# precice/dealii-adapter

Hardware: AMD Instinct MI355X
Metric: DoF-updates/sec per Newmark step (assembly+CG), 3D Q2 ~5M DoFs (higher is better)
Workload: dtype f64

## Files before the change

dealii-adapter_amd/csrc/mi_ctx.cpp:

```cpp
#include <hip/hip_runtime.h>
#include <rccl/rccl.h>

#include <algorithm>
#include <chrono>
#include <cmath>
#include <cstdarg>
#include <cstdio>
#include <cstdlib>
#include <cstring>
#include <functional>
#include <string>
#include <vector>

#include "mi_internal.h"

namespace mi_detail
{
  std::string g_create_error;

  enum
  {
    SC_RZ0 = 0,
    SC_RZ1 = 1,
    SC_TOL = 2,
// ... 120 lines not shown
      L.begin[c] = int32_t(m.ncells);
    L.ncol = m.ncolours;
    const int npc = m.npc, np1 = m.np1;
    for (int64_t pos = 0; pos < m.ncells; ++pos)
      {
        int col = 0;
        for (int c = 1; c < 8; ++c)
          col += pos >= L.begin[c] ? 1 : 0;
        const mi::CellLatticeRow &R = rows[size_t(col)];
        const uint32_t r   = uint32_t(pos - L.begin[col]);
        const uint32_t rz  = uint32_t((uint64_t(r) * R.magic_mxy) >> 42);
        const uint32_t rem = r - rz * uint32_t(R.mxy);
        const uint32_t ry  = uint32_t((uint64_t(rem) * R.magic_mx) >> 42);
        const uint32_t rx  = rem - ry * uint32_t(R.mx);
        const int32_t  n0  = R.base + int32_t(rx) * L.sx + int32_t(ry) * L.sy + int32_t(rz) * L.sz;
        for (int a = 0; a < npc; ++a)
          {
            const int i = a % np1, j = (a / np1) % np1, k = a / (np1 * np1);
            if (m.conn[size_t(pos) * npc + a] != n0 + i + j * L.nn0 + k * L.nn01)
              return mi::CellLattice{};
          }
      }
    return L;
  }

  mi::AsmParams asm_params(mi_ctx *c)
  {
    mi::AsmParams p{};
    static const bool asm_lat = mi::exp_env("MI_ASM_CELL_LATTICE") && atoi(mi::exp_env("MI_ASM_CELL_LATTICE")) != 0;
    if (asm_lat)
      p.lat = c->lat;
    p.conn   = c->d_conn;
    p.cverts = c->d_cverts;
    p.off    = c->d_off;
    p.rowinfo = reinterpret_cast<const int2 *>(c->d_rowinfo);
    p.cmask  = c->d_cmask;
    p.tab1d  = c->d_tab;
    p.u      = c->vec(MI_V_TOTAL_DISPLACEMENT);
    p.du     = c->vec(MI_V_SOLUTION_DELTA);
    p.acc    = c->vec(MI_V_ACCELERATION);
    p.stress = c->vec(MI_V_EXTERNAL_STRESS);
    p.rhs    = c->vec(MI_V_SYSTEM_RHS);
    p.vals   = c->d_vals;
    p.zero_blk  = uint32_t(c->mesh.nvalblocks() + 1);
    p.trash_blk = uint32_t(c->mesh.nvalblocks() + 2);
    p.mu     = c->mat.mu;
// ... 143 lines not shown

  int element_form(const mi_ctx *c)
  {
    if (!c->ke_valid)
      return 0;
    if (c->d_qrec_q3)
      return 2;
    if (c->d_qrec && (c->ebe == 2 || !c->d_ke))
      return 2;
    return c->d_ke ? 1 : 0;
  }

  bool smoother_runs_q27(const mi_ctx *c)
  {
    return c->smoother_points == 3 && c->qrec27_valid && element_form(c) == 2 && c->mf_slots && c->d_mf_yc &&
           !c->active_sell_vals && (c->mf_fine || (c->ebe != 0 && c->precond_storage == 64)) &&
           !(c->smoother_precision == 32 && c->qrec32_valid);
  }

  bool mf_gather_fusable(const mi_ctx *c)
  {
    return element_form(c) == 2 && c->ebe == 2 && c->mf_slots && c->d_mf_yc && c->precond_storage == 64 &&
           !c->active_sell_vals && c->d_dinv_blk;
  }

  mi::MfParams mf_params(const mi_ctx *c)
  {
    mi::MfParams f{};
    f.conn = c->d_conn, f.first = c->d_node_first, f.cmask = c->d_cmask, f.cverts = c->d_cverts, f.cellbox = c->d_cellbox;
    f.tab1d = c->d_tab, f.tab27 = c->d_tab27, f.lat = c->lat, f.qrec27 = c->d_qrec27;
    f.mu = c->mat.mu, f.kappa = c->kappa, f.mass = c->alpha[1] * c->mat.rho;
    return f;
  }

  void enqueue_spmv(mi_ctx *c, const double *x, double *y, const double *dotv, double *partials, const int32_t *done,
                    int part, bool smoother, const ChebFusion *cheb)
  {
    const int  kind       = element_form(c);
    const bool mf_all     = c->mf_fine && !c->active_sell_vals;
    const bool ebe_for_cg = dotv && (c->cg_operator == 1 || mf_all) && kind && !c->active_sell_vals && !cheb;
    const bool cheb_ok    = !cheb || (cheb->inplace && smoother && mf_gather_fusable(c));
    if (ebe_for_cg || (kind && cheb_ok && !dotv && !c->active_sell_vals &&
                       (mf_all || (smoother ? (c->ebe != 0 && c->precond_storage == 64) : (c->spmv_variant == 4 || c->unassembled_now)))))
      {
        const bool q3  = c->d_qrec_q3 != nullptr;
        const bool q27 = smoother && !ebe_for_cg && smoother_runs_q27(c);
// ... 61 lines not shown
                    return;
                  }
                layers(0, zlo, false);
                layers(zhi, nzl, false);
              }
            else if (q3)
              {
                const int t = sample ? tic(c0, MI_T_EBE_LAUNCH, true) : -1;
                mi::launch_mf_spmv_q3(f, int32_t(c->mesh.ncells), c->stream, t >= 0 ? c0->stamps[size_t(t)].a : nullptr,
                                      t >= 0 ? c0->stamps[size_t(t)].b : nullptr);
              }
            else if (q27)
              {
                const int t = sample ? tic(c0, MI_T_EBE_LAUNCH, true) : -1;
                mi::launch_mf_spmv27(f, int32_t(c->mesh.ncells), c->stream, t >= 0 ? c0->stamps[size_t(t)].a : nullptr,
                                     t >= 0 ? c0->stamps[size_t(t)].b : nullptr);
              }
            else
              {
                const int t = sample ? tic(c0, MI_T_EBE_LAUNCH, true) : -1;
                mi::launch_mf_spmv(f, 0, int32_t(c->mesh.ncells), c->stream, t >= 0 ? c0->stamps[size_t(t)].a : nullptr,
                                   t >= 0 ? c0->stamps[size_t(t)].b : nullptr);
              }
            if (cheb && cheb->xnext)
              mi::launch_mf_gather_cheb3(f, cheb->b, cheb->dinv6, cheb->xprev, x, cheb->xnext, cheb->c1, cheb->c2, c->own0 / 3,
                                         c->own_n / 3, c->stream);
            else if (cheb)
              mi::launch_mf_gather_cheb(f, cheb->b, cheb->dinv, cheb->d, const_cast<double *>(x), y, cheb->c1, cheb->c2,
                                        c->own0 / 3, c->own_n / 3, c->stream);
            else if (ebe_for_cg)
              mi::launch_mf_gather_dot(f, int64_t(c->mesh.nnodes) * 3, dotv, partials, c->grid_gdot, c->own0, c->own_n, c->stream);
            else
              mi::launch_mf_gather(f, int64_t(c->mesh.nnodes) * 3, c->stream);
          }
        else
        for (int col = 0; col < c->mesh.ncolours; ++col)
          {
            const int32_t cnt = int32_t(c->mesh.colour_begin[col + 1] - c->mesh.colour_begin[col]);
            const int     t   = (sample && cnt > 0) ? tic(c0, MI_T_EBE_LAUNCH, true) : -1;
            if (kind == 2)
              mi::launch_mf_spmv(f, c->mesh.colour_begin[col], cnt, c->stream, t >= 0 ? c0->stamps[size_t(t)].a : nullptr,
                                 t >= 0 ? c0->stamps[size_t(t)].b : nullptr);
            else
              mi::launch_ebe_spmv(e, c->mesh.colour_begin[col], cnt, c->stream, t >= 0 ? c0->stamps[size_t(t)].a : nullptr,
                                  t >= 0 ? c0->stamps[size_t(t)].b : nullptr);
          }
        if (ebe_for_cg && !one_launch)
          mi::launch_dot_partials(dotv + c->own0, y + c->own0, c->own_n, partials, c->grid_vec, c->stream);
        return;
      }
    if (c->spmv_variant == 3 || c->spmv_variant == 4 || c->active_sell_vals)
      {
        refresh_vals32(c);
        mi::SellParams p   = sell_params(c, x, y, dotv, partials, done);
        if (smoother && c->precond_storage == 32 && c->d_sell_vals32 && !c->active_sell_vals)
          p.vals32 = c->d_sell_vals32;
// ... 367 lines not shown
      layout = 1;
    c->slots_layout = layout;
    if (layout)
      {
        src.resize(dst.size());
        std::vector<int32_t> place(dst.size());
        for (size_t k = 0; k < dst.size(); ++k)
          place[k] = int32_t(k);
        if (layout == 2)
          for (int col = 0; col < c->lat.ncol; ++col)
            {
              const mi::CellLatticeRow &R  = c->lat_rows_host[size_t(col)];
              const int64_t             b0 = c->lat.begin[col], b1 = c->lat.begin[col + 1];
              for (int64_t e = b0; e < b1; ++e)
                {
                  const int64_t r = e - b0, row = r / R.mx, rx = r - row * R.mx;
                  for (int a = 0; a < 27; ++a)
                    place[size_t(e) * 27 + a] = int32_t((b0 + row * R.mx) * 27 + int64_t(a / 3) * 3 * R.mx + rx * 3 + a % 3);
                }
            }
        for (size_t k = 0; k < dst.size(); ++k)
          src[size_t(dst[k])] = place[k];
        dst = place;
      }
    const bool cell_major = layout != 0;
    int rc = upload(c, &c->d_mf_dst, dst);
    if (rc == MI_OK)
      rc = upload(c, &c->d_mf_slot_base, base);
    if (rc == MI_OK && cell_major)
      rc = upload(c, &c->d_mf_src, src);
    if (rc)
      return rc;
    if (!c->d_mf_yc)
      HIPCHK(c, hipMalloc((void **)&c->d_mf_yc, size_t(nc) * npc * 3 * sizeof(double)));
    
    return MI_OK;
  }

  int alloc_records27(mi_ctx *c)
  {
    if (c->d_qrec27 || c->smoother_points != 3)
      return MI_OK;
    mi::Tables1D t3;
    t3.build(2, 3);
    const int rc = upload(c, &c->d_tab27, t3.packed());
    if (rc)
// ... 1877 lines not shown
            {
              const int rq = alloc_point_records(m);
              if (rq)
                return rq;
            }
          if (!m->d_node_first)
            {
              const int rc = upload(m, &m->d_node_first, m->mesh.node_first);
              if (rc)
                return rc;
            }
          m->ebe      = value;
          m->ke_valid = false;
        }
      else if (k == "mg_scale_lmax_percent" && value >= 10 && value <= 400)
        {
          if (m == c->team->members[0])
            mg_scale_estimates(*c->team, 0.01 * value);
        }
      else if (k == "mf_single_launch" && (value == 0 || value == 1))
        m->mf_slots = value;
      else if (k == "xcd_remap" && (value == 0 || value == 1))
        m->xcd_remap = value;
      else if (k == "cell_lattice" && (value == 0 || value == 1))
        m->lat = value ? m->lat_built : mi::CellLattice{};
      else if (k == "sell_unroll" && value >= -2 && value <= 8 && value != 0)
        m->sell_unroll = value;
      else if (k == "spmv_grid" && value >= 1 && value + m->grid_spmv_bnd <= MAX_PART)
        {
          m->split_int = m->split_bnd = false;
          if (m->mesh.sell_nslices_interior > 0)
            m->grid_spmv_int = value;
          else
            m->grid_spmv_bnd = value;
          m->grid_spmv = m->grid_spmv_int + m->grid_spmv_bnd;
        }
      else if (k == "sell_icol" && (value == 0 || value == 1))
        m->sell_icol = value;
      else if (k == "small_cg" && (value == 0 || value == 1))
        m->small_cg = value;
      else if (k == "halo_overlap" && (value == 0 || value == 1))
        c->team->overlap = value;
      else if (k == "asm_variant" && ((value >= 0 && value <= 2) || value == 9))
        m->asm_variant = value;
      else if (k == "mg_refresh_every" && value >= 1 && value <= 1000)
        m->mg_refresh_every = value;
// ... 89 lines not shown
               0;
  else if (k == "mf_single_launch")
    *value = (m->mf_slots && m->d_mf_yc) ? 1 : 0;
  else if (k == "fine_level")
    *value = m->mf_fine;
  else if (k == "mf_diag_lag")
    *value = m->mf_diag_lag;
  else if (k == "smoother_quadrature")
    *value = m->smoother_points;
  else if (k == "smoother_quadrature_active")
    *value = smoother_runs_q27(m) ? 3 : 4;
  else if (k == "experiments")
#ifdef MI_EXPERIMENTS
    *value = 1;
#else
    *value = 0;
#endif
  else if (k == "sell_icol")
    *value = m->sell_icol;
  else if (k == "asm_variant")
    *value = m->asm_variant;
  else if (k == "cell_lattice")
    *value = m->lat.ncol > 0 ? 1 : 0;
  else if (k == "cut_axis")
    *value = c->team->size > 1 ? c->team->amap.ext_axis[c->team->dim - 1] + 1 : 0;
  else if (k == "cg_speculate")
    *value = m->cg_speculate;
  else if (k == "smoother_precision")
    *value = m->smoother_precision;
  else if (k == "cg_single_reduction")
    *value = m->cg_single_reduction;
  else if (k == "mg_distributed_levels")
    *value = mg_distributed_levels(m);
  else if (k == "cg_single_reduction_active")
    *value = (m->cg_single_reduction == 1 || (m->cg_single_reduction < 0 && c->team->size > 1)) ? 1 : 0;
  else if (k == "cg_speculate_margin")
    *value = m->cg_speculate_margin;
  else if (k == "halo_skip")
    *value = c->team->halo_skip;
  else if (k == "precond")
    *value = m->precond;
  else if (k == "spmv_variant")
    *value = m->spmv_variant;
  else if (k == "count_scalar_allreduce")
    *value = int(c->team->n_scalar_allreduce);
  else if (k == "count_scalar_allreduce_cg")
// ... 174 lines not shown
```

dealii-adapter_amd/csrc/mi_internal.h:

```cpp
#pragma once
#include <hip/hip_runtime.h>

#include <cstdint>
#include <functional>
#include <memory>
#include <string>
#include <vector>

#include "../../include/mi_elasticity.h"
#include "mi_kernels.h"
#include "mi_mesh.hpp"

namespace mi_detail
{
  constexpr int MAX_PART = 16384;
  constexpr int CG_BATCH = 16;

  enum
  {
    W_R = 0,
    W_P,
    W_Q,
    W_DINV,
    W_Z,
// ... 88 lines not shown
  bool      want_dinv_blk = false;
  double   *d_ke = nullptr;
  uint32_t *d_node_first = nullptr;
  float    *d_qrec32 = nullptr;
  int       smoother_precision = 64;
  int       smoother_points = 3;
  double   *d_qrec27 = nullptr;
  double   *d_tab27  = nullptr;
  bool      qrec27_valid = false;
  int       spmv_as_smoother = 0;
  bool      qrec32_valid = false;
  double   *d_qrec = nullptr;
  double   *d_mf_yc = nullptr;
  int32_t  *d_mf_dst = nullptr;
  int32_t  *d_mf_slot_base = nullptr;
  int32_t  *d_mf_src = nullptr;
  int       slots_layout = 0;
  int       slots_cell_major = -1;
  int       mf_slots = 1;
  mi::CellLattice lat;
  mi::CellLattice lat_built;
  mi::CellLatticeRow *d_lat_rows = nullptr;
  std::vector<mi::CellLatticeRow> lat_rows_host;
  double   *d_cellbox = nullptr;
  bool      ke_valid = false;
  int64_t   ebe_products = 0;
  static constexpr int NPRED = 4;
  double   *d_pred[NPRED][2] = {}, *d_pred_saved[NPRED][2] = {};
  int       pred_count[NPRED] = {}, pred_count_saved[NPRED] = {}, solves_this_step = 0;
  int       cg_operator = 0;
  int       cg_warm_start = 0;
  int       cg_fused_dot = 1;
  int       correct_face_F = 0;
  int       cg_r0_unassembled = 1;
  bool      unassembled_now = false;
  int64_t   mg_dist_nodes = -1;
  int64_t   mg_coarsest = -1, mg_dense = -1;
  int       cg_single_reduction = -1;
  int       cg_speculate_margin = 0;
  int       cg_speculate = 1;
  int       pred_its[NPRED] = {};
  int       mf_fine = 0;
  double   *d_qrec_q3 = nullptr;
  int       mf_point_slots = 1;
  int       mf_diag_lag = 0;
  bool      mf_diag_fresh = false;
// ... 50 lines not shown
  bool                  mg_stale = true;
  bool                  mg_force = true;
  int                   asm_variant = 0;
  int                   asm_box_geometry = 1;
  int                   mg_lag   = 1;
  int                   mg_refresh_every = 8, mg_steps_since_refresh = 0, mg_its_ref = 0;
  int64_t               n_mg_refresh = 0;

  double *vec(int which) { return d_vecs + size_t(which) * size_t(n); }
  double *work(int which) { return d_work + size_t(which) * size_t(n); }
  double *part(int which) { return d_part + size_t(which) * mi_detail::MAX_PART; }
};

namespace mi_detail
{
  int  fail(mi_ctx *c, int code, const char *fmt, ...);
  int  tic(mi_ctx *c, int cls, bool ext = false);
  void toc(mi_ctx *c, int id);
  int  sync(mi_ctx *c);
  int            direct_prepare(mi_ctx *c);
  int            direct_factor_solve(mi_ctx *c, const double *vals, const double *b, double *x, bool factor, bool solve);
  void           refresh_vals32(mi_ctx *c);
  int            element_form(const mi_ctx *c);
  bool           mf_gather_fusable(const mi_ctx *c);
  mi::SellParams sell_params(mi_ctx *c, const double *x, double *y, const double *dotv, double *partials,
                             const int32_t *done);
  void enqueue_spmv(mi_ctx *c, const double *x, double *y, const double *dotv, double *partials, const int32_t *done,
                    int part = 0, bool smoother = false, const ChebFusion *cheb = nullptr);
  int  set_precond_storage(mi_ctx *c, int bits);
  int  cg_run(mi_ctx *c, int x_id, int b_id, double tol, int64_t max_it, int *its, double *res, bool x_is_zero = false,
              bool scale_start = false,
              int expected_its = 0);
  int  team_size(const mi_ctx *c);
  void linear_destroy(mi_ctx *c);
  int  create_member(Team &T, const mi_mesh_desc *md, const mi_material_desc *mat, const mi_newmark_desc *nm, int rank,
                     mi_ctx **out);
  void destroy_team(Team *T);
  int  enqueue_assembly(mi_ctx *c, bool residual_only = false);
  int  ensure_element_tangents(mi_ctx *c);
  int  mg_setup(mi_ctx *c);
  void mg_reset_estimates(Team &T);
  void mg_scale_estimates(Team &T, double f);
  void mg_destroy(mi_ctx *c);
  int  mg_update(Team &T);
  int  mg_distributed_levels(const mi_ctx *c);
  int  mg_apply(Team &T);
// ... 39 lines not shown
```

dealii-adapter_amd/csrc/mi_kernels.h:

```cpp
#pragma once
#include <hip/hip_runtime.h>
#include <stdint.h>

#include <stdlib.h>

namespace mi
{
#ifdef MI_EXPERIMENTS
  inline const char *exp_env(const char *name) { return getenv(name); }
#else
  inline const char *exp_env(const char *) { return nullptr; }
#endif

  struct CellLatticeRow
  {
    int32_t  mx, mxy, base, pz;
    uint64_t magic_mx, magic_mxy;
  };
  struct CellLattice
  {
    int32_t               ncol = 0;
    int32_t               begin[9] = {};
    int32_t               sx = 0, sy = 0, sz = 0, nn0 = 0, nn01 = 0;
    const CellLatticeRow *rows = nullptr;
  };

  struct AsmParams
  {
    const int32_t  *conn;
    const double   *cverts;
    const uint16_t *off;
    const int2     *rowinfo;
    const uint8_t  *cmask;
    const double   *tab1d;
    const double   *u, *du, *acc, *stress;
    double         *rhs;
    double         *vals;
    uint32_t        zero_blk, trash_blk;
    double          mu, kappa, rho, alpha1;
    double          body[3];
    int64_t         cell_begin;
    int32_t         cell_count;
    int32_t         variant;
    int32_t         residual_only;
    double         *qrec;
    float          *qrec32;
    int32_t         axmap;
    double         *inverted;
// ... 151 lines not shown
    double       *f_old, *v, *d, *v_old, *d_old, *rhs, *w;
    double        theta, dt;
    int64_t       n;
  };

  void launch_linear_rhs_prepare(const LinearParams &p, hipStream_t s);
  void launch_linear_rhs_finish(int dim, const LinearParams &p, const double *mv, const double *kw,
                                const uint8_t *cmask, hipStream_t s);
  void launch_linear_update_displacement(const LinearParams &p, hipStream_t s);
  int  launch_assemble_cells(int dim, int degree, const AsmParams &p, hipStream_t s);
  int  launch_neumann_faces(int dim, int degree, const AsmParams &p, const int32_t *faces, int face_begin,
                            int face_count, hipStream_t s);
  void launch_neumann_gather(int dim, const double *slots, const int32_t *node_ids, const int32_t *start, const int32_t *src,
                             const uint8_t *cmask, double *rhs, int nnodes_if, hipStream_t s);
  void launch_spmv(int dim, const SpmvParams &p, int grid, hipStream_t s, int variant, int maxrow);
  void launch_sell_spmv(int dim, const SellParams &p, int grid, hipStream_t s, int unroll);
  void set_next_sell_launch_events(hipEvent_t start, hipEvent_t stop);
  void launch_ebe_spmv(const EbeParams &p, int64_t cell_begin, int32_t cell_count, hipStream_t s,
                       hipEvent_t ev_start = nullptr, hipEvent_t ev_stop = nullptr);
  void launch_mf_spmv(const MfParams &p, int64_t cell_begin, int32_t cell_count, hipStream_t s,
                      hipEvent_t ev_start = nullptr, hipEvent_t ev_stop = nullptr);
  void launch_mf_spmv27(const MfParams &p, int32_t cell_count, hipStream_t s, hipEvent_t ev_start = nullptr, hipEvent_t ev_stop = nullptr);
  void launch_mf_records27(const MfParams &p, const double *u, const double *du, double *rec27, int32_t cell_count, hipStream_t s);
  void launch_mf_gather(const MfParams &p, int64_t ndofs, hipStream_t s);
  void launch_mf_gather_dot(const MfParams &p, int64_t ndofs, const double *dotv, double *partials, int grid, int64_t own0,
                            int64_t own_n, hipStream_t s);
  void launch_mf_diag(const MfParams &p, double *slots6, int32_t cell_count, hipStream_t s);
  constexpr int MF_Q3_QS = 128;
  void launch_mf_records_q3(const MfParams &p, const double *u, const double *du, double *rec, int32_t cell_count, hipStream_t s);
  void launch_mf_spmv_q3(const MfParams &p, int32_t cell_count, hipStream_t s, hipEvent_t ev_start = nullptr, hipEvent_t ev_stop = nullptr);
  void launch_mf_diag_q3(const MfParams &p, double *slots6, int32_t cell_count, hipStream_t s);
  void launch_point_pass_slots(const AsmParams &p, hipStream_t s);
  void launch_residual_gather(const double *slots3, const int32_t *slot_base, const int32_t *slot_src, const uint8_t *cmask, double *rhs,
                              int64_t ndofs, hipStream_t s);
  void launch_mf_diag_gather(const double *slots6, const int32_t *slot_base, const int32_t *slot_src, const uint8_t *cmask,
                             const int32_t *diagpos, double *blk, double *dinv, double *dinv_blk, double *sym6, int64_t nnodes, hipStream_t s);
  void launch_mf_gather_cheb3(const MfParams &p, const double *b, const double *dinv6, const double *xprev, const double *xcur,
                              double *xnext, double c1, double c2, int64_t node0, int64_t nnodes, hipStream_t s);
  void launch_mf_gather_cheb(const MfParams &p, const double *b, const double *dinv, double *d, double *xio, double *yres,
                             double c1, double c2, int64_t node0, int64_t nnodes, hipStream_t s);
  int  launch_dense_inverse_from_sell(int dim, const SellParams &p, int n, double *out, hipStream_t s);
  void launch_dense_apply(const double *inv, const double *b, double *x, int n, hipStream_t s);
  constexpr int BAND_NB = 16, BAND_MAXH = 512;
  void launch_band_extract(int dim, const SellParams &p, const int32_t *bperm, double *band, int hbw, hipStream_t s);
  int  launch_band_cholesky_solve(int dim, double *band, int n, int hbw, const int32_t *bperm, int nnodes, const double *b,
                                  double *x, double *work, int32_t *flag, bool factor, bool solve, hipStream_t s);
  constexpr int SELL_SPLIT_MAX_SLICES = 160;
  constexpr int SELL_WPB = 3;
  constexpr int EBE_NBLK = 378;
  void launch_vals_to_f32(const double *vals, float *vals32, int64_t n, hipStream_t s);
  void launch_sell_build_cols(const SellParams &p, const int32_t *rowptr, const int32_t *bsr_col, int32_t *sell_col,
                              hipStream_t s);
  void launch_dot_partials(const double *a, const double *b, int64_t n, double *part, int grid, hipStream_t s);
  void launch_finish_sum(const double *part, int n, double *out, hipStream_t s);
  void launch_cheb4_start(double *x, double *d, double *r, const double *b, const double *q, const double *dinv,
                          double s0, int64_t n, hipStream_t s);
  void launch_cheb4_step(double *x, double *d, double *r, const double *q, const double *dinv, double beta, double ca,
                         double cb, int64_t n, hipStream_t s);
  void launch_extract_dinv_blk(int dim, const double *vals, const int32_t *diagpos, double *dinv, double *sym6, int64_t nnodes,
                               hipStream_t s);
  void launch_gather_diag_blocks(int dim, const double *vals, const int32_t *diagpos, double *out, int64_t nnodes, hipStream_t s);
  void launch_blk_apply(int dim, double *out, const double *a, const double *dinv, int64_t nnodes, hipStream_t s);
  void launch_cheb_step_blk(int dim, double *x, double *d, const double *b, const double *q, const double *dinv,
// ... 41 lines not shown
```

dealii-adapter_amd/csrc/mi_kernels.hip:

```cpp
#include <hip/hip_runtime.h>
#include <hip/hip_ext.h>
#include <stdint.h>

#include <type_traits>

#include "mi_kernels.h"

namespace mi
{
  __device__ __forceinline__ int64_t imin64(int64_t a, int64_t b)
  {
    return a < b ? a : b;
  }

  __device__ __forceinline__ double wave_sum(double v)
  {
#pragma unroll
    for (int o = 32; o >= 1; o >>= 1)
      v += __shfl_xor(v, o, 64);
    return v;
  }

  template <int CTRL, int ROW_MASK, int BANK_MASK>
  __device__ __forceinline__ double dpp_add(double v)
// ... 2643 lines not shown
      {
        const int64_t n = g / 3;
        const int     c = int(g - n * 3);
        double        s;
        if ((prm.cmask[n] >> c) & 1)
          {
            const int32_t dp = prm.diagpos[n];
            s                = dp >= 0 ? prm.vals[int64_t(dp) * 9 + c * 4] * prm.x[g] : 0.0;
          }
        else
          {
            const int32_t b0 = prm.slot_base[n], b1 = prm.slot_base[n + 1];
            s                = mf_slot_sum(prm, b0, b1, c);
          }
        prm.y[g] = s;
        if (g >= own0 && g < own0 + own_n)
          acc = fma(dotv[g], s, acc);
      }
    acc = block_sum<256>(acc, s_red);
    if (threadIdx.x == 0)
      partials[blockIdx.x] = acc;
  }

  constexpr int DG_NF = 20;
#define MF_DIAG_POINT(BOX_, MO_, MI_, tx_, qx_, qy_, qz_, store_, o_)                                          \
  double Finv[9], tau[6], tiso[6], cII, cS, Ji[9], detJ, M[9];                                                  \
  neo_hooke_from_F<3>(rec, det3x3(rec), rec[9], rec[10], prm.mu, prm.kappa, Finv, tau, tiso, cII, cS);          \
  mf_geometry<BOX_>(prm, cell, tx_, qx_, qy_, qz_, Ji, detJ);                                                   \
  MF_M(BOX_, MO_, MI_)                                                                                          \
  const double w  = detJ * wq;                                                                                  \
  const double pv = tau[0] - tiso[0];                                                    \
  if (store_)                                                                                                   \
    {                                                                                                           \
      double *o = (o_);                                                                                         \
      _Pragma("unroll") for (int k_ = 0; k_ < 9; ++k_) o[k_] = M[k_];                                           \
      _Pragma("unroll") for (int k_ = 0; k_ < 6; ++k_) o[9 + k_] = tau[k_];                                     \
      o[15] = 0.5 * w * (cII + 0.5 * cS + (4.0 / 3.0) * pv);                                                    \
      o[16] = (2.0 / 3.0) * w;                                                                                  \
      o[17] = 0.5 * cS * w;                                                                                     \
      o[18] = w;                                                                                                \
      o[19] = prm.mass * w;                                                                                     \
    }
#define MF_DIAG_ACCUMULATE                                                      \
  {                                                                             \
    double g[3], tg[3], v[3];                                                   \
    _Pragma("unroll") for (int j_ = 0; j_ < 3; ++j_)                            \
// ... 3285 lines not shown
    if (n > DENSE_BIG_MAX)
      return -1;
    if (n > DENSE_MAX)
      {
        if (dim == 3)
          hipLaunchKernelGGL((dense_inverse_from_sell_big<3>), dim3(1), dim3(1024), 0, s, p, n, out);
        else
          hipLaunchKernelGGL((dense_inverse_from_sell_big<2>), dim3(1), dim3(1024), 0, s, p, n, out);
      }
    else if (dim == 3)
      hipLaunchKernelGGL((dense_inverse_from_sell<3>), dim3(1), dim3(256), 0, s, p, n, out);
    else
      hipLaunchKernelGGL((dense_inverse_from_sell<2>), dim3(1), dim3(256), 0, s, p, n, out);
    return 0;
  }
  void launch_dense_apply(const double *inv, const double *b, double *x, int n, hipStream_t s)
  {
    if (n > DENSE_MAX)
      hipLaunchKernelGGL(dense_apply_big, dim3((n + 15) / 16), dim3(256), 0, s, inv, b, x, n);
    else
      hipLaunchKernelGGL(dense_apply, dim3(1), dim3(128), 0, s, inv, b, x, n);
  }

  void launch_mf_gather_cheb(const MfParams &p, const double *b, const double *dinv, double *d, double *xio, double *yres,
                             double c1, double c2, int64_t node0, int64_t nnodes, hipStream_t s)
  {
    if (nnodes <= 0)
      return;
    hipLaunchKernelGGL(mf_gather_cheb, dim3(int((nnodes + 63) / 64)), dim3(192), 0, s, p, b, dinv, d, xio, yres, c1, c2,
                       node0, nnodes);
  }
  void launch_mf_gather_cheb3(const MfParams &p, const double *b, const double *dinv6, const double *xprev, const double *xcur,
                              double *xnext, double c1, double c2, int64_t node0, int64_t nnodes, hipStream_t s)
  {
    if (nnodes <= 0)
      return;
    hipLaunchKernelGGL(mf_gather_cheb3, dim3(int((nnodes + 63) / 64)), dim3(192), 0, s, p, b, dinv6, xprev, xcur, xnext, c1, c2,
                       node0, nnodes);
  }
  void launch_mf_gather(const MfParams &p, int64_t ndofs, hipStream_t s)
  {
    hipLaunchKernelGGL(mf_gather, dim3(int((ndofs + 255) / 256)), dim3(256), 0, s, p, ndofs);
  }
  void launch_mf_gather_dot(const MfParams &p, int64_t ndofs, const double *dotv, double *partials, int grid, int64_t own0,
                            int64_t own_n, hipStream_t s)
  {
    hipLaunchKernelGGL(mf_gather_dot, dim3(grid), dim3(256), 0, s, p, ndofs, dotv, partials, own0, own_n);
  }
  void launch_point_pass_slots(const AsmParams &p, hipStream_t s)
  {
    if (p.cell_count <= 0)
      return;
    AsmParams q = p;
    q.xcd_chunk = (p.cell_count + 7) / 8;
    hipLaunchKernelGGL((assemble_q2sf<true, true>), dim3(q.xcd_chunk * 8), dim3(64), 0, s, q);
  }
  void launch_residual_gather(const double *slots3, const int32_t *slot_base, const int32_t *slot_src, const uint8_t *cmask, double *rhs,
                              int64_t ndofs, hipStream_t s)
  {
    hipLaunchKernelGGL(residual_gather, dim3(int((ndofs + 255) / 256)), dim3(256), 0, s, slots3, slot_base, slot_src, cmask, rhs, ndofs);
  }
  void launch_mf_spmv27(const MfParams &p, int32_t cell_count, hipStream_t s, hipEvent_t ev_start, hipEvent_t ev_stop)
  {
    if (cell_count <= 0)
      return;
    MfParams q  = p;
    q.count     = cell_count;
    q.xcd_chunk = ((cell_count + 1) / 2 + 7) / 8;
    auto *kern  = q.lat.ncol > 0 ? (q.cellbox ? mf_spmv27<true, true> : mf_spmv27<false, true>) :
                                   (q.cellbox ? mf_spmv27<true, false> : mf_spmv27<false, false>);
// ... 356 lines not shown
```

Baseline: 52.36 million.

## Compute gather slot indices from structured lattice instead of CSR slot lists

Adds a SlotLattice descriptor, built on the host and checked against the existing slot_base/slot_src lists. The matrix-free gather kernels (plain, dot, Chebyshev, Chebyshev3) use it to derive each node's up-to-8 contributing cell slots arithmetically from its (i,j,k) lattice coordinate, which removes the indirect index-list loads. An optional tiled variant walks x-lines in 2x2 (j,k) groups of nodes so that neighbouring threads read neighbouring yc slots. The change adds integer arithmetic per node and new kernel variants, and it falls back to the list path when validation fails or the partition is not plane-aligned.

```diff
diff --git a/dealii-adapter_amd/csrc/mi_ctx.cpp b/dealii-adapter_amd/csrc/mi_ctx.cpp
--- a/dealii-adapter_amd/csrc/mi_ctx.cpp
+++ b/dealii-adapter_amd/csrc/mi_ctx.cpp
@@ -166,6 +166,37 @@
           }
       }
     return L;
+  }
+
+  mi::SlotLattice build_slot_lattice(const mi::HostMesh &m, const mi::CellLattice &L, const std::vector<mi::CellLatticeRow> &rows)
+  {
+    mi::SlotLattice S{};
+    if (L.ncol <= 0 || m.dim != 3 || m.p != 2 || rows.size() < size_t(L.ncol) || m.nnodes >= (int64_t(1) << 31) ||
+        m.ncells * 27 >= (int64_t(1) << 31))
+      return S;
+    for (int v = 0; v < 8; ++v)
+      S.begin[v] = -1, S.mx[v] = 1, S.mxy[v] = 1;
+    int last = -1;
+    for (int c = 0; c < L.ncol; ++c)
+      {
+        int ci[3];
+        mi::HostMesh::split(m.cell_orig[size_t(L.begin[c])], m.reps, 3, ci);
+        const int v = (ci[0] & 1) | ((ci[1] & 1) << 1) | ((ci[2] & 1) << 2);
+        if (v <= last)
+          return mi::SlotLattice{};
+        last        = v;
+        S.begin[v]  = L.begin[c];
+        S.mx[v]     = rows[size_t(c)].mx;
+        S.mxy[v]    = rows[size_t(c)].mxy;
+      }
+    for (int d = 0; d < 3; ++d)
+      S.nc[d] = m.reps[d];
+    S.nn0        = L.nn0;
+    S.nn01       = L.nn01;
+    S.magic_nn0  = ~uint64_t(0) / uint64_t(S.nn0) + 1;
+    S.magic_nn01 = ~uint64_t(0) / uint64_t(S.nn01) + 1;
+    S.ncol       = L.ncol;
+    return S;
   }
 
   mi::AsmParams asm_params(mi_ctx *c)
@@ -355,6 +386,15 @@
   {
     return element_form(c) == 2 && c->ebe == 2 && c->mf_slots && c->d_mf_yc && c->precond_storage == 64 &&
            !c->active_sell_vals && c->d_dinv_blk;
+  }
+
+  int gather_lattice_mode(const mi_ctx *c)
+  {
+    if (c->gather_lattice == 0 || c->slot_lat.ncol == 0 || c->lat.ncol == 0 || c->slots_layout != 1)
+      return 0;
+    const int     want  = c->gather_lattice < 0 ? 2 : c->gather_lattice;
+    const int64_t plane = c->slot_lat.nn01, n0 = c->own0 / 3, nn = c->own_n / 3;
+    return (want >= 2 && nn > 0 && n0 % plane == 0 && nn % plane == 0) ? want : 1;
   }
 
   mi::MfParams mf_params(const mi_ctx *c)
@@ -462,16 +502,19 @@
                 mi::launch_mf_spmv(f, 0, int32_t(c->mesh.ncells), c->stream, t >= 0 ? c0->stamps[size_t(t)].a : nullptr,
                                    t >= 0 ? c0->stamps[size_t(t)].b : nullptr);
               }
+            const int                gmode = gather_lattice_mode(c);
+            const mi::SlotLattice   *sl    = gmode ? &c->slot_lat : nullptr;
+            const bool               tw    = gmode >= 2;
             if (cheb && cheb->xnext)
               mi::launch_mf_gather_cheb3(f, cheb->b, cheb->dinv6, cheb->xprev, x, cheb->xnext, cheb->c1, cheb->c2, c->own0 / 3,
-                                         c->own_n / 3, c->stream);
+                                         c->own_n / 3, c->stream, sl, tw);
             else if (cheb)
               mi::launch_mf_gather_cheb(f, cheb->b, cheb->dinv, cheb->d, const_cast<double *>(x), y, cheb->c1, cheb->c2,
-                                        c->own0 / 3, c->own_n / 3, c->stream);
+                                        c->own0 / 3, c->own_n / 3, c->stream, sl, tw);
             else if (ebe_for_cg)
-              mi::launch_mf_gather_dot(f, int64_t(c->mesh.nnodes) * 3, dotv, partials, c->grid_gdot, c->own0, c->own_n, c->stream);
+              mi::launch_mf_gather_dot(f, int64_t(c->mesh.nnodes) * 3, dotv, partials, c->grid_gdot, c->own0, c->own_n, c->stream, sl);
             else
-              mi::launch_mf_gather(f, int64_t(c->mesh.nnodes) * 3, c->stream);
+              mi::launch_mf_gather(f, int64_t(c->mesh.nnodes) * 3, c->stream, sl);
           }
         else
         for (int col = 0; col < c->mesh.ncolours; ++col)
@@ -885,6 +928,22 @@
         for (size_t k = 0; k < dst.size(); ++k)
           src[size_t(dst[k])] = place[k];
         dst = place;
+      }
+    c->slot_lat = mi::SlotLattice{};
+    if (layout == 1 && npc == 27)
+      {
+        mi::SlotLattice S = build_slot_lattice(c->mesh, c->lat_built, c->lat_rows_host);
+        for (int64_t n = 0; n < nn && S.ncol > 0; ++n)
+          {
+            int32_t   list[8];
+            const int cnt = mi::slot_lattice_list(S, uint32_t(n), list);
+            bool      same = cnt == base[size_t(n) + 1] - base[size_t(n)];
+            for (int q = 0; q < cnt && same; ++q)
+              same = list[q] == src[size_t(base[size_t(n)]) + q];
+            if (!same)
+              S = mi::SlotLattice{};
+          }
+        c->slot_lat = S;
       }
     const bool cell_major = layout != 0;
     int rc = upload(c, &c->d_mf_dst, dst);
@@ -2808,6 +2867,8 @@
         m->mf_slots = value;
       else if (k == "xcd_remap" && (value == 0 || value == 1))
         m->xcd_remap = value;
+      else if (k == "mf_gather_lattice" && value >= -1 && value <= 2)
+        m->gather_lattice = value;
       else if (k == "cell_lattice" && (value == 0 || value == 1))
         m->lat = value ? m->lat_built : mi::CellLattice{};
       else if (k == "sell_unroll" && value >= -2 && value <= 8 && value != 0)
@@ -2943,6 +3004,10 @@
     *value = m->asm_variant;
   else if (k == "cell_lattice")
     *value = m->lat.ncol > 0 ? 1 : 0;
+  else if (k == "mf_gather_lattice")
+    *value = m->gather_lattice;
+  else if (k == "mf_gather_lattice_active")
+    *value = gather_lattice_mode(m);
   else if (k == "cut_axis")
     *value = c->team->size > 1 ? c->team->amap.ext_axis[c->team->dim - 1] + 1 : 0;
   else if (k == "cg_speculate")
diff --git a/dealii-adapter_amd/csrc/mi_internal.h b/dealii-adapter_amd/csrc/mi_internal.h
--- a/dealii-adapter_amd/csrc/mi_internal.h
+++ b/dealii-adapter_amd/csrc/mi_internal.h
@@ -134,6 +134,8 @@
   mi::CellLattice lat_built;
   mi::CellLatticeRow *d_lat_rows = nullptr;
   std::vector<mi::CellLatticeRow> lat_rows_host;
+  mi::SlotLattice slot_lat;
+  int       gather_lattice = -1;
   double   *d_cellbox = nullptr;
   bool      ke_valid = false;
   int64_t   ebe_products = 0;
@@ -230,6 +232,7 @@
   int            direct_factor_solve(mi_ctx *c, const double *vals, const double *b, double *x, bool factor, bool solve);
   void           refresh_vals32(mi_ctx *c);
   int            element_form(const mi_ctx *c);
+  int            gather_lattice_mode(const mi_ctx *c);
   bool           mf_gather_fusable(const mi_ctx *c);
   mi::SellParams sell_params(mi_ctx *c, const double *x, double *y, const double *dotv, double *partials,
                              const int32_t *done);
diff --git a/dealii-adapter_amd/csrc/mi_kernels.h b/dealii-adapter_amd/csrc/mi_kernels.h
--- a/dealii-adapter_amd/csrc/mi_kernels.h
+++ b/dealii-adapter_amd/csrc/mi_kernels.h
@@ -24,6 +24,70 @@
     int32_t               sx = 0, sy = 0, sz = 0, nn0 = 0, nn01 = 0;
     const CellLatticeRow *rows = nullptr;
   };
+
+  struct SlotLattice
+  {
+    int32_t  ncol = 0;
+    int32_t  nc[3] = {};
+    int32_t  nn0 = 0, nn01 = 0;
+    uint64_t magic_nn0 = 0, magic_nn01 = 0;
+    int32_t  begin[8] = {}, mx[8] = {}, mxy[8] = {};
+  };
+  __host__ __device__ inline uint32_t slot_lattice_div(const uint32_t n, const uint64_t magic)
+  {
+#if defined(__HIP_DEVICE_COMPILE__)
+    return uint32_t(__umul64hi(uint64_t(n), magic));
+#else
+    return uint32_t((static_cast<unsigned __int128>(n) * magic) >> 64);
+#endif
+  }
+  __host__ __device__ inline void slot_lattice_ijk(const SlotLattice &L, const uint32_t n, int32_t &i, int32_t &j, int32_t &k)
+  {
+    const uint32_t kk = slot_lattice_div(n, L.magic_nn01), rem = n - kk * uint32_t(L.nn01);
+    const uint32_t jj = slot_lattice_div(rem, L.magic_nn0);
+    i = int32_t(rem - jj * uint32_t(L.nn0)), j = int32_t(jj), k = int32_t(kk);
+  }
+  template <int P>
+  __host__ __device__ inline void slot_lattice_axis(const int32_t i, const int32_t ncells, int32_t &r, int32_t &l, bool &ok)
+  {
+    const int32_t h = i >> 1, odd = i & 1;
+    const bool    at_h = (h & 1) == P;
+    r  = (h - (at_h ? 0 : 1)) >> 1;
+    l  = at_h ? odd : 2;
+    ok = at_h ? h < ncells : (odd == 0 && h >= 1);
+  }
+  __host__ __device__ inline void slot_lattice_slots(const SlotLattice &L, const int32_t i, const int32_t j, const int32_t k,
+                                                     int32_t slot[8])
+  {
+    int32_t rx[2], lx[2], ry[2], ly[2], rz[2], lz[2];
+    bool    okx[2], oky[2], okz[2];
+    slot_lattice_axis<0>(i, L.nc[0], rx[0], lx[0], okx[0]);
+    slot_lattice_axis<1>(i, L.nc[0], rx[1], lx[1], okx[1]);
+    slot_lattice_axis<0>(j, L.nc[1], ry[0], ly[0], oky[0]);
+    slot_lattice_axis<1>(j, L.nc[1], ry[1], ly[1], oky[1]);
+    slot_lattice_axis<0>(k, L.nc[2], rz[0], lz[0], okz[0]);
+    slot_lattice_axis<1>(k, L.nc[2], rz[1], lz[1], okz[1]);
+#pragma unroll
+    for (int v = 0; v < 8; ++v)
+      {
+        const int  px = v & 1, py = (v >> 1) & 1, pz = v >> 2;
+        const bool ok = okx[px] && oky[py] && okz[pz] && L.begin[v] >= 0;
+        const int32_t pos = L.begin[v] + rz[pz] * L.mxy[v] + ry[py] * L.mx[v] + rx[px];
+        slot[v] = (pos * 27 + lx[px] + 3 * ly[py] + 9 * lz[pz]) | (ok ? 0 : -1);
+      }
+  }
+  __host__ __device__ inline int slot_lattice_list(const SlotLattice &L, const uint32_t n, int32_t list[8])
+  {
+    int32_t i, j, k, slot[8];
+    slot_lattice_ijk(L, n, i, j, k);
+    slot_lattice_slots(L, i, j, k, slot);
+    int cnt = 0;
+#pragma unroll
+    for (int v = 0; v < 8; ++v)
+      if (slot[v] >= 0)
+        list[cnt++] = slot[v];
+    return cnt;
+  }
 
   struct AsmParams
   {
@@ -221,9 +285,9 @@
                       hipEvent_t ev_start = nullptr, hipEvent_t ev_stop = nullptr);
   void launch_mf_spmv27(const MfParams &p, int32_t cell_count, hipStream_t s, hipEvent_t ev_start = nullptr, hipEvent_t ev_stop = nullptr);
   void launch_mf_records27(const MfParams &p, const double *u, const double *du, double *rec27, int32_t cell_count, hipStream_t s);
-  void launch_mf_gather(const MfParams &p, int64_t ndofs, hipStream_t s);
+  void launch_mf_gather(const MfParams &p, int64_t ndofs, hipStream_t s, const SlotLattice *sl = nullptr);
   void launch_mf_gather_dot(const MfParams &p, int64_t ndofs, const double *dotv, double *partials, int grid, int64_t own0,
-                            int64_t own_n, hipStream_t s);
+                            int64_t own_n, hipStream_t s, const SlotLattice *sl = nullptr);
   void launch_mf_diag(const MfParams &p, double *slots6, int32_t cell_count, hipStream_t s);
   constexpr int MF_Q3_QS = 128;
   void launch_mf_records_q3(const MfParams &p, const double *u, const double *du, double *rec, int32_t cell_count, hipStream_t s);
@@ -235,9 +299,11 @@
   void launch_mf_diag_gather(const double *slots6, const int32_t *slot_base, const int32_t *slot_src, const uint8_t *cmask,
                              const int32_t *diagpos, double *blk, double *dinv, double *dinv_blk, double *sym6, int64_t nnodes, hipStream_t s);
   void launch_mf_gather_cheb3(const MfParams &p, const double *b, const double *dinv6, const double *xprev, const double *xcur,
-                              double *xnext, double c1, double c2, int64_t node0, int64_t nnodes, hipStream_t s);
+                              double *xnext, double c1, double c2, int64_t node0, int64_t nnodes, hipStream_t s,
+                              const SlotLattice *sl = nullptr, bool tiles = false);
   void launch_mf_gather_cheb(const MfParams &p, const double *b, const double *dinv, double *d, double *xio, double *yres,
-                             double c1, double c2, int64_t node0, int64_t nnodes, hipStream_t s);
+                             double c1, double c2, int64_t node0, int64_t nnodes, hipStream_t s, const SlotLattice *sl = nullptr,
+                             bool tiles = false);
   int  launch_dense_inverse_from_sell(int dim, const SellParams &p, int n, double *out, hipStream_t s);
   void launch_dense_apply(const double *inv, const double *b, double *x, int n, hipStream_t s);
   constexpr int BAND_NB = 16, BAND_MAXH = 512;
diff --git a/dealii-adapter_amd/csrc/mi_kernels.hip b/dealii-adapter_amd/csrc/mi_kernels.hip
--- a/dealii-adapter_amd/csrc/mi_kernels.hip
+++ b/dealii-adapter_amd/csrc/mi_kernels.hip
@@ -2689,6 +2689,246 @@
       partials[blockIdx.x] = acc;
   }
 
+  __device__ __forceinline__ void mf_slot_load_lattice(const MfParams &prm, const int32_t (&slot)[8], const int c, double (&v)[8])
+  {
+#pragma unroll
+    for (int p = 0; p < 8; ++p)
+      v[p] = slot[p] >= 0 ? prm.yc[int64_t(slot[p]) * 3 + c] : 0.0;
+  }
+  __device__ __forceinline__ double mf_slot_add_lattice(const int32_t (&slot)[8], const double (&v)[8])
+  {
+    double s    = 0.0;
+    bool   have = false;
+#pragma unroll
+    for (int p = 0; p < 8; ++p)
+      if (slot[p] >= 0)
+        {
+          s    = have ? s + v[p] : v[p];
+          have = true;
+        }
+    return s;
+  }
+
+  __global__ __launch_bounds__(256) void mf_gather_lat(MfParams prm, SlotLattice sl, int64_t ndofs)
+  {
+    const int64_t g = int64_t(blockIdx.x) * 256 + threadIdx.x;
+    if (g >= ndofs)
+      return;
+    const int64_t n = g / 3;
+    const int     c = int(g - n * 3);
+    int32_t       i, j, k, slot[8];
+    double        v[8];
+    slot_lattice_ijk(sl, uint32_t(n), i, j, k);
+    slot_lattice_slots(sl, i, j, k, slot);
+    const uint8_t cm = prm.cmask[n];
+    mf_slot_load_lattice(prm, slot, c, v);
+    double s = mf_slot_add_lattice(slot, v);
+    if ((cm >> c) & 1)
+      {
+        const int32_t dp = prm.diagpos[n];
+        s                = dp >= 0 ? prm.vals[int64_t(dp) * 9 + c * 4] * prm.x[g] : 0.0;
+      }
+    prm.y[g] = s;
+  }
+
+  __global__ __launch_bounds__(256) void mf_gather_dot_lat(MfParams prm, SlotLattice sl, int64_t ndofs,
+                                                           const double *__restrict__ dotv, double *partials, int64_t own0,
+                                                           int64_t own_n)
+  {
+    __shared__ double s_red[4];
+    double            acc = 0.0;
+    const int64_t     per = ((ndofs + gridDim.x - 1) / gridDim.x + 255) / 256 * 256;
+    const int64_t     g0 = int64_t(blockIdx.x) * per, g1 = imin64(ndofs, g0 + per);
+    for (int64_t g = g0 + threadIdx.x; g < g1; g += 256)
+      {
+        const int64_t n = g / 3;
+        const int     c = int(g - n * 3);
+        int32_t       i, j, k, slot[8];
+        double        v[8];
+        slot_lattice_ijk(sl, uint32_t(n), i, j, k);
+        slot_lattice_slots(sl, i, j, k, slot);
+        const uint8_t cm   = prm.cmask[n];
+        const bool    own  = g >= own0 && g < own0 + own_n;
+        const double  dv   = own ? dotv[g] : 0.0;
+        mf_slot_load_lattice(prm, slot, c, v);
+        double s = mf_slot_add_lattice(slot, v);
+        if ((cm >> c) & 1)
+          {
+            const int32_t dp = prm.diagpos[n];
+            s                = dp >= 0 ? prm.vals[int64_t(dp) * 9 + c * 4] * prm.x[g] : 0.0;
+          }
+        prm.y[g] = s;
+        if (own)
+          acc = fma(dv, s, acc);
+      }
+    acc = block_sum<256>(acc, s_red);
+    if (threadIdx.x == 0)
+      partials[blockIdx.x] = acc;
+  }
+
+  constexpr int MF_TILE_SEG = 128, MF_TILE_W = 64;
+  template <int W>
+  struct MfGatherMap
+  {
+    static constexpr int NT = W ? 12 * W : 192;
+    int32_t j = 0, k = 0, x0 = 0, xi = 0;
+    bool    line_in = false;
+    __device__ __forceinline__ MfGatherMap(const SlotLattice &sl, const int m, const int64_t node0, const int64_t nnodes)
+    {
+      if constexpr (W > 0)
+        {
+          const int32_t k0 = int32_t(slot_lattice_div(uint32_t(node0), sl.magic_nn01));
+          const int32_t k1 = k0 + int32_t(slot_lattice_div(uint32_t(nnodes), sl.magic_nn01));
+          const int     line = m / W;
+          xi      = m % W;
+          j       = int32_t(blockIdx.y) * 2 + (line & 1);
+          k       = ((k0 >> 1) + int32_t(blockIdx.z)) * 2 + (line >> 1);
+          x0      = int32_t(blockIdx.x) * MF_TILE_SEG;
+          line_in = j <= 2 * sl.nc[1] && k >= k0 && k < k1;
+        }
+    }
+    static __device__ __forceinline__ int steps() { return W ? MF_TILE_SEG / W : 1; }
+    __device__ __forceinline__ bool node(const SlotLattice &sl, const int st, const int m, const int64_t node0, const int64_t nnodes,
+                                         int64_t &n, int32_t &i, int32_t &jj, int32_t &kk) const
+    {
+      if constexpr (W > 0)
+        {
+          i  = x0 + st * W + xi;
+          jj = j, kk = k;
+          const bool in = line_in && i < sl.nn0;
+          n             = in ? int64_t(i) + int64_t(sl.nn0) * j + int64_t(sl.nn01) * k : node0;
+          return in;
+        }
+      else
+        {
+          const int64_t nl = int64_t(blockIdx.x) * 64 + m;
+          const bool    in = nl < nnodes;
+          n                = in ? node0 + nl : node0;
+          slot_lattice_ijk(sl, uint32_t(n), i, jj, kk);
+          return in;
+        }
+    }
+    __device__ __forceinline__ bool more(const SlotLattice &sl, const int st) const
+    {
+      return W > 0 && st + 1 < steps() && x0 + (st + 1) * W < sl.nn0;
+    }
+  };
+
+  template <int W>
+  __global__ __launch_bounds__(MfGatherMap<W>::NT) void mf_gather_cheb_lat(MfParams prm, SlotLattice sl, const double *__restrict__ b,
+                                                                          const double *__restrict__ dinv, double *d, double *xio,
+                                                                          double *yres, double c1, double c2, int64_t node0,
+                                                                          int64_t nnodes)
+  {
+    constexpr int NT = MfGatherMap<W>::NT;
+    __shared__ double s_res[2][NT];
+    const int            ld = threadIdx.x, c = ld % 3, m = ld / 3;
+    const MfGatherMap<W> map(sl, m, node0, nnodes);
+    for (int st = 0;; ++st)
+      {
+        int64_t    n;
+        int32_t    i, j, k, slot[8];
+        double     v[8];
+        const bool in = map.node(sl, st, m, node0, nnodes, n, i, j, k);
+        const int64_t g = n * 3 + c;
+        double     res = 0.0, a0 = 0.0, a1 = 0.0, a2 = 0.0, dold = 0.0, xold = 0.0;
+        if (in)
+          {
+            slot_lattice_slots(sl, i, j, k, slot);
+            const uint8_t cm = prm.cmask[n];
+            const double  bv = b[g];
+            if (d)
+              {
+                a0 = dinv[g * 3], a1 = dinv[g * 3 + 1], a2 = dinv[g * 3 + 2];
+                dold = c1 != 0.0 ? d[g] : 0.0;
+                xold = xio[g];
+              }
+            mf_slot_load_lattice(prm, slot, c, v);
+            double q = mf_slot_add_lattice(slot, v);
+            if ((cm >> c) & 1)
+              q = prm.vals[int64_t(prm.diagpos[n]) * 9 + c * 4] * prm.x[g];
+            res = bv - q;
+          }
+        if (!d)
+          {
+            if (in)
+              yres[g] = res;
+          }
+        else
+          {
+            double *sr = s_res[st & 1];
+            sr[ld]     = res;
+            __syncthreads();
+            if (in)
+              {
+                const int r0 = (ld / 3) * 3;
+                double    s  = 0.0;
+                s += a0 * sr[r0];
+                s += a1 * sr[r0 + 1];
+                s += a2 * sr[r0 + 2];
+                const double dn = (c1 != 0.0 ? c1 * dold : 0.0) + c2 * s;
+                d[g]            = dn;
+                xio[g]          = xold + dn;
+              }
+          }
+        if (!map.more(sl, st))
+          break;
+      }
+  }
+
+  template <int W>
+  __global__ __launch_bounds__(MfGatherMap<W>::NT) void mf_gather_cheb3_lat(MfParams prm, SlotLattice sl, const double *__restrict__ b,
+                                                                           const double *__restrict__ dinv6, const double *xprev,
+                                                                           const double *__restrict__ xcur, double *xnext,
+                                                                           double c1, double c2, int64_t node0, int64_t nnodes)
+  {
+    constexpr int NT = MfGatherMap<W>::NT;
+    __shared__ double s_res[2][NT];
+    const int            ld = threadIdx.x, c = ld % 3, m = ld / 3;
+    const MfGatherMap<W> map(sl, m, node0, nnodes);
+    for (int st = 0;; ++st)
+      {
+        int64_t    n;
+        int32_t    i, j, k, slot[8];
+        double     v[8];
+        const bool in = map.node(sl, st, m, node0, nnodes, n, i, j, k);
+        const int64_t g = n * 3 + c;
+        double     res = 0.0, xc = 0.0, xp = 0.0, a0 = 0.0, a1 = 0.0, a2 = 0.0;
+        if (in)
+          {
+            slot_lattice_slots(sl, i, j, k, slot);
+            const uint8_t cm = prm.cmask[n];
+            const double *q6 = dinv6 + n * 6;
+            a0               = q6[c == 0 ? 0 : (c == 1 ? 3 : 4)];
+            a1               = q6[c == 0 ? 3 : (c == 1 ? 1 : 5)];
+            a2               = q6[c == 0 ? 4 : (c == 1 ? 5 : 2)];
+            xc               = xcur[g];
+            xp               = (c1 != 0.0 && xprev) ? xprev[g] : 0.0;
+            const double bv  = b[g];
+            mf_slot_load_lattice(prm, slot, c, v);
+            double q = mf_slot_add_lattice(slot, v);
+            if ((cm >> c) & 1)
+              q = prm.vals[int64_t(prm.diagpos[n]) * 9 + c * 4] * xc;
+            res = bv - q;
+          }
+        double *sr = s_res[st & 1];
+        sr[ld]     = res;
+        __syncthreads();
+        if (in)
+          {
+            const int r0 = (ld / 3) * 3;
+            double    s  = 0.0;
+            s += a0 * sr[r0];
+            s += a1 * sr[r0 + 1];
+            s += a2 * sr[r0 + 2];
+            const double dn = (c1 != 0.0 ? c1 * (xc - xp) : 0.0) + c2 * s;
+            xnext[g]        = xc + dn;
+          }
+        if (!map.more(sl, st))
+          break;
+      }
+  }
+
   constexpr int DG_NF = 20;
 #define MF_DIAG_POINT(BOX_, MO_, MI_, tx_, qx_, qy_, qz_, store_, o_)                                          \
   double Finv[9], tau[6], tiso[6], cII, cS, Ji[9], detJ, M[9];                                                  \
@@ -6020,30 +6260,56 @@
       hipLaunchKernelGGL(dense_apply, dim3(1), dim3(128), 0, s, inv, b, x, n);
   }
 
+  static dim3 mf_tile_grid(const SlotLattice &sl, int64_t node0, int64_t nnodes)
+  {
+    const int64_t k0 = node0 / sl.nn01, k1 = k0 + nnodes / sl.nn01;
+    return dim3(unsigned((sl.nn0 + MF_TILE_SEG - 1) / MF_TILE_SEG), unsigned(sl.nc[1] + 1), unsigned(((k1 - 1) >> 1) - (k0 >> 1) + 1));
+  }
   void launch_mf_gather_cheb(const MfParams &p, const double *b, const double *dinv, double *d, double *xio, double *yres,
-                             double c1, double c2, int64_t node0, int64_t nnodes, hipStream_t s)
+                             double c1, double c2, int64_t node0, int64_t nnodes, hipStream_t s, const SlotLattice *sl, bool tiles)
   {
     if (nnodes <= 0)
       return;
-    hipLaunchKernelGGL(mf_gather_cheb, dim3(int((nnodes + 63) / 64)), dim3(192), 0, s, p, b, dinv, d, xio, yres, c1, c2,
-                       node0, nnodes);
+    if (sl && sl->ncol > 0 && tiles)
+      hipLaunchKernelGGL(mf_gather_cheb_lat<MF_TILE_W>, mf_tile_grid(*sl, node0, nnodes), dim3(MfGatherMap<MF_TILE_W>::NT), 0, s, p,
+                         *sl, b, dinv, d, xio, yres, c1, c2, node0, nnodes);
+    else if (sl && sl->ncol > 0)
+      hipLaunchKernelGGL(mf_gather_cheb_lat<0>, dim3(int((nnodes + 63) / 64)), dim3(192), 0, s, p, *sl, b, dinv, d, xio, yres, c1, c2,
+                         node0, nnodes);
+    else
+      hipLaunchKernelGGL(mf_gather_cheb, dim3(int((nnodes + 63) / 64)), dim3(192), 0, s, p, b, dinv, d, xio, yres, c1, c2,
+                         node0, nnodes);
   }
   void launch_mf_gather_cheb3(const MfParams &p, const double *b, const double *dinv6, const double *xprev, const double *xcur,
-                              double *xnext, double c1, double c2, int64_t node0, int64_t nnodes, hipStream_t s)
+                              double *xnext, double c1, double c2, int64_t node0, int64_t nnodes, hipStream_t s,
+                              const SlotLattice *sl, bool tiles)
   {
     if (nnodes <= 0)
       return;
-    hipLaunchKernelGGL(mf_gather_cheb3, dim3(int((nnodes + 63) / 64)), dim3(192), 0, s, p, b, dinv6, xprev, xcur, xnext, c1, c2,
-                       node0, nnodes);
-  }
-  void launch_mf_gather(const MfParams &p, int64_t ndofs, hipStream_t s)
-  {
-    hipLaunchKernelGGL(mf_gather, dim3(int((ndofs + 255) / 256)), dim3(256), 0, s, p, ndofs);
+    if (sl && sl->ncol > 0 && tiles)
+      hipLaunchKernelGGL(mf_gather_cheb3_lat<MF_TILE_W>, mf_tile_grid(*sl, node0, nnodes), dim3(MfGatherMap<MF_TILE_W>::NT), 0, s, p,
+                         *sl, b, dinv6, xprev, xcur, xnext, c1, c2, node0, nnodes);
+    else if (sl && sl->ncol > 0)
+      hipLaunchKernelGGL(mf_gather_cheb3_lat<0>, dim3(int((nnodes + 63) / 64)), dim3(192), 0, s, p, *sl, b, dinv6, xprev, xcur, xnext,
+                         c1, c2, node0, nnodes);
+    else
+      hipLaunchKernelGGL(mf_gather_cheb3, dim3(int((nnodes + 63) / 64)), dim3(192), 0, s, p, b, dinv6, xprev, xcur, xnext, c1, c2,
+                         node0, nnodes);
+  }
+  void launch_mf_gather(const MfParams &p, int64_t ndofs, hipStream_t s, const SlotLattice *sl)
+  {
+    if (sl && sl->ncol > 0)
+      hipLaunchKernelGGL(mf_gather_lat, dim3(int((ndofs + 255) / 256)), dim3(256), 0, s, p, *sl, ndofs);
+    else
+      hipLaunchKernelGGL(mf_gather, dim3(int((ndofs + 255) / 256)), dim3(256), 0, s, p, ndofs);
   }
   void launch_mf_gather_dot(const MfParams &p, int64_t ndofs, const double *dotv, double *partials, int grid, int64_t own0,
-                            int64_t own_n, hipStream_t s)
-  {
-    hipLaunchKernelGGL(mf_gather_dot, dim3(grid), dim3(256), 0, s, p, ndofs, dotv, partials, own0, own_n);
+                            int64_t own_n, hipStream_t s, const SlotLattice *sl)
+  {
+    if (sl && sl->ncol > 0)
+      hipLaunchKernelGGL(mf_gather_dot_lat, dim3(grid), dim3(256), 0, s, p, *sl, ndofs, dotv, partials, own0, own_n);
+    else
+      hipLaunchKernelGGL(mf_gather_dot, dim3(grid), dim3(256), 0, s, p, ndofs, dotv, partials, own0, own_n);
   }
   void launch_point_pass_slots(const AsmParams &p, hipStream_t s)
   {
```

Result: faster. 53.45 million, median of 6 (+2.1%).
